# Aedelon/ProteinBERT-PyTorch-Replication

Hardware: AMD Instinct MI355X
Metric: sequences/sec (whole node) ProteinBERT pretrain L=512 at 1/2/4/8 MI355X (higher is better)
Workload: dtype bf16; 1 GPU; global_batch=2048, per_gpu_batch=2048, seq_len=512, parallelism=dp1, impl=hip, hip_graph=False

## Files before the change

proteinbert_pytorch_replication_amd/ops/csrc/lhead.hip:

```cpp
#include "mfma.h"

using namespace pbx;
typedef unsigned short bf16_t;

namespace {
constexpr int CH = 128;
constexpr int SB = 16;
constexpr int PT = 32;
constexpr int VP = 32;

__device__ __forceinline__ void stage_wo(unsigned char* wos, float* bo_s, const float* __restrict__ wo,
                                        const float* __restrict__ bo, int V) {
  for (int idx = threadIdx.x; idx < VP * 16; idx += blockDim.x) {
    const int v = idx >> 4, c8 = idx & 15;
    float e[8] = {0, 0, 0, 0, 0, 0, 0, 0};
    if (v < V) {
      const float4 a = *reinterpret_cast<const float4*>(wo + v * CH + c8 * 8);
      const float4 b = *reinterpret_cast<const float4*>(wo + v * CH + c8 * 8 + 4);
      e[0] = a.x; e[1] = a.y; e[2] = a.z; e[3] = a.w; e[4] = b.x; e[5] = b.y; e[6] = b.z; e[7] = b.w;
    }
    *reinterpret_cast<uint4*>(wos + swz256(v, c8)) = packq8(e);
  }
  if (threadIdx.x < VP) bo_s[threadIdx.x] = threadIdx.x < V ? bo[threadIdx.x] : 0.f;
}

__device__ __forceinline__ void tile_of(int L, int& b0, int& p0, int& chunk) {
  const int TP = (L + PT - 1) / PT;
  chunk = blockIdx.x / TP;
  b0 = chunk * SB;
  p0 = (blockIdx.x - chunk * TP) * PT;
}

__global__ void __launch_bounds__(512) lhead_logits_kernel(const bf16_t* __restrict__ h, const float* __restrict__ wo,
                                                           const float* __restrict__ bo, float* __restrict__ Z,
                                                           float2* __restrict__ part, int B, int L, int V) {
  extern __shared__ __attribute__((aligned(16))) unsigned char smem[];
  unsigned char* wos = smem;
  float* bo_s = reinterpret_cast<float*>(smem + VP * 256);
  float (*zt)[PT][VP + 1] = reinterpret_cast<float (*)[PT][VP + 1]>(bo_s + VP);
  const int tid = threadIdx.x, lane = tid & 63, w = tid >> 6;
  const int r = lane & 31, hh = lane >> 5;
  int b0, p0, chunk;
  tile_of(L, b0, p0, chunk);
  stage_wo(wos, bo_s, wo, bo, V);
  __syncthreads();
  bf16x8 wf[8];
#pragma unroll
  for (int kk = 0; kk < 8; ++kk) wf[kk] = lds_frag(wos, swz256(r, kk * 2 + hh));
  const float bv = bo_s[r];
#pragma unroll
  for (int si = 0; si < 2; ++si) {
    const int sl = 2 * w + si, b = b0 + sl;
    const int pos = p0 + r;
    const bool okrow = b < B && pos < L;
    const size_t row = (size_t)min(b, B - 1) * L + min(pos, L - 1);
    bf16x8 hf[8];
#pragma unroll
    for (int kk = 0; kk < 8; ++kk) hf[kk] = *reinterpret_cast<const bf16x8*>(h + row * CH + kk * 16 + 8 * hh);
    f32x16_t acc = zero16();
#pragma unroll
    for (int kk = 0; kk < 8; ++kk) acc = mfma32(hf[kk], wf[kk], acc);
#pragma unroll
    for (int e = 0; e < 16; ++e) {
      const int pl = (e & 3) + 8 * (e >> 2) + 4 * hh;
      const int pp = p0 + pl;
      const float z = acc[e] + bv;
      zt[sl][pl][r] = z;
      if (b < B && pp < L) Z[((size_t)b * L + pp) * VP + r] = r < V ? z : 0.f;
    }
    (void)okrow;
  }
  __syncthreads();
  {
    const int pl = tid >> 4, v0 = (tid & 15) * 2;
    const int pp = p0 + pl;
    const int nb = min(SB, B - b0);
    if (pp < L) {
#pragma unroll
      for (int j = 0; j < 2; ++j) {
        const int v = v0 + j;
        float m = -3.0e38f;
        for (int s = 0; s < nb; ++s) m = fmaxf(m, zt[s][pl][v]);
        float se = 0.f;
        for (int s = 0; s < nb; ++s) se += __expf(zt[s][pl][v] - m);
        part[((size_t)chunk * L + pp) * VP + v] = make_float2(m, se);
      }
    }
  }
}

__global__ void __launch_bounds__(256) lhead_fold_kernel(const float2* __restrict__ part, int nchunks, int L,
                                                         float2* __restrict__ out, int mode) {
  __shared__ float2 red[4][64];
  const int il = threadIdx.x & 63, cg = threadIdx.x >> 6;
  const int i = blockIdx.x * 64 + il;
  const bool ok = i < L * VP;
  float m = -3.0e38f, sum = 0.f;
  if (ok) {
    for (int c = cg; c < nchunks; c += 4) {
      const float2 p = part[(size_t)c * L * VP + i];
      if (mode != 1) {
        const float mn = fmaxf(m, p.x);
        sum = sum * __expf(m - mn) + p.y * __expf(p.x - mn);
        m = mn;
      } else {
        sum += p.x;
      }
    }
  }
  red[cg][il] = make_float2(m, sum);
  __syncthreads();
  if (cg != 0 || !ok) return;
  if (mode != 1) {
    float mm = red[0][il].x;
#pragma unroll
    for (int k = 1; k < 4; ++k) mm = fmaxf(mm, red[k][il].x);
    float ss = 0.f;
#pragma unroll
    for (int k = 0; k < 4; ++k) ss += red[k][il].y * __expf(red[k][il].x - mm);
    out[i] = make_float2(mm, mode == 2 ? ss : ss > 0.f ? 1.0f / ss : 0.f);
  } else {
    out[i] = make_float2(red[0][il].y + red[1][il].y + red[2][il].y + red[3][il].y, 0.f);
  }
}

struct RowTerms {
  float P[16], G[16];
  float loss;
};
__device__ __forceinline__ RowTerms row_terms(const float* __restrict__ Z, const float2* ms, size_t row, int pl,
                                              int hh, int V, bool ok, int yv, float coef) {
  RowTerms t;
  float zv[16];
  {
    const float4* zp0 = reinterpret_cast<const float4*>(Z + row * VP + 8 * hh);
    const float4* zp1 = reinterpret_cast<const float4*>(Z + row * VP + 16 + 8 * hh);
    const float4 a = zp0[0], b = zp0[1], c = zp1[0], d = zp1[1];
    const float tmp[16] = {a.x, a.y, a.z, a.w, b.x, b.y, b.z, b.w, c.x, c.y, c.z, c.w, d.x, d.y, d.z, d.w};
#pragma unroll
    for (int j = 0; j < 16; ++j) zv[j] = tmp[j];
  }
  float e[16], se = 0.f, py = 0.f;
#pragma unroll
  for (int j = 0; j < 16; ++j) {
    const int v = (j < 8 ? 0 : 16) + 8 * hh + (j & 7);
    const float2 s = ms[pl * VP + v];
    const bool inv = v < V;
    t.P[j] = inv ? __expf(zv[j] - s.x) * s.y : 0.f;
    e[j] = inv ? __expf(t.P[j]) : 0.f;
    se += e[j];
    py += v == yv ? t.P[j] : 0.f;
  }
  se += __shfl_xor(se, 32, 64);
  const float rse = 1.0f / se;
#pragma unroll
  for (int j = 0; j < 16; ++j) {
    const int v = (j < 8 ? 0 : 16) + 8 * hh + (j & 7);
    t.G[j] = ok ? coef * (e[j] * rse - (v == yv ? 1.f : 0.f)) : 0.f;
  }
  t.loss = ok ? ((hh == 0 ? __logf(se) : 0.f) - py) : 0.f;
  return t;
}

__global__ void __launch_bounds__(512) lhead_ce_kernel(const float* __restrict__ Z, const float2* __restrict__ MS,
                                                       const long long* __restrict__ y, const float* __restrict__ wl,
                                                       float2* __restrict__ tpart, float* __restrict__ loss_part,
                                                       int B, int L, int V, float inv_bl) {
  __shared__ float2 ms[PT * VP];
  __shared__ float gp[8][PT][VP + 1];
  __shared__ float red[8];
  const int tid = threadIdx.x, lane = tid & 63, w = tid >> 6;
  const int r = lane & 31, hh = lane >> 5;
  int b0, p0, chunk;
  tile_of(L, b0, p0, chunk);
  for (int i = tid; i < PT * VP; i += 512) {
    const int pp = min(p0 + i / VP, L - 1);
    ms[i] = MS[(size_t)pp * VP + (i % VP)];
  }
  __syncthreads();
  float acc[16];
#pragma unroll
  for (int j = 0; j < 16; ++j) acc[j] = 0.f;
  float lsum = 0.f;
#pragma unroll
  for (int si = 0; si < 2; ++si) {
    const int b = b0 + 2 * w + si, pos = p0 + r;
    const bool ok = b < B && pos < L;
    const size_t row = (size_t)min(b, B - 1) * L + min(pos, L - 1);
    const int yv = (int)y[row];
    const float wgt = ok ? wl[row] : 0.f;
    const RowTerms t = row_terms(Z, ms, row, r, hh, V, ok, yv, wgt * inv_bl);
    lsum += wgt * t.loss;
#pragma unroll
    for (int j = 0; j < 16; ++j) acc[j] += t.G[j] * t.P[j];
  }
#pragma unroll
  for (int j = 0; j < 16; ++j) gp[w][r][(j < 8 ? 0 : 16) + 8 * hh + (j & 7)] = acc[j];
  lsum = wave_reduce_sum(lsum);
  if (lane == 0) red[w] = lsum;
  __syncthreads();
  for (int i = tid; i < PT * VP; i += 512) {
    const int pl = i / VP, v = i % VP;
    if (p0 + pl < L) {
      float s = 0.f;
#pragma unroll
      for (int ww = 0; ww < 8; ++ww) s += gp[ww][pl][v];
      tpart[((size_t)chunk * L + p0 + pl) * VP + v] = make_float2(s, 0.f);
    }
  }
  if (tid == 0) {
    float s = 0.f;
#pragma unroll
    for (int ww = 0; ww < 8; ++ww) s += red[ww];
    loss_part[blockIdx.x] = s * inv_bl;
  }
}

__global__ void __launch_bounds__(512) lhead_grad_kernel(const float* __restrict__ Z, const float2* __restrict__ MS,
                                                         const float2* __restrict__ T, const long long* __restrict__ y,
                                                         const float* __restrict__ wl, const float* __restrict__ wo,
                                                         const float* __restrict__ bo, bf16_t* __restrict__ dh,
                                                         bf16_t* __restrict__ dz, float* __restrict__ dbo_part, int B,
                                                         int L, int V, float inv_bl) {
  extern __shared__ __attribute__((aligned(16))) unsigned char smem[];
  unsigned char* ot = smem;
  unsigned char* wos = smem + 8 * PT * 256;
  float2* ms = reinterpret_cast<float2*>(wos + VP * 256);
  float* ts = reinterpret_cast<float*>(ms + PT * VP);
  float* bo_s = ts + PT * VP;
  float (*dbr)[VP] = reinterpret_cast<float (*)[VP]>(bo_s + VP);
  const int tid = threadIdx.x, lane = tid & 63, w = tid >> 6;
  const int r = lane & 31, hh = lane >> 5;
  const int q = tr_q(lane), tc = tr_c(lane);
  int b0, p0, chunk;
  tile_of(L, b0, p0, chunk);
  stage_wo(wos, bo_s, wo, bo, V);
  for (int i = tid; i < PT * VP; i += 512) {
    const int pp = min(p0 + i / VP, L - 1);
    ms[i] = MS[(size_t)pp * VP + (i % VP)];
    ts[i] = T[(size_t)pp * VP + (i % VP)].x;
  }
  __syncthreads();
  float dba[16];
#pragma unroll
  for (int j = 0; j < 16; ++j) dba[j] = 0.f;
  unsigned char* myot = ot + w * PT * 256;
#pragma unroll 1
  for (int si = 0; si < 2; ++si) {
    const int b = b0 + 2 * w + si, pos = p0 + r;
    const bool ok = b < B && pos < L;
    const size_t row = (size_t)min(b, B - 1) * L + min(pos, L - 1);
    const int yv = (int)y[row];
    const float wgt = ok ? wl[row] : 0.f;
    const RowTerms t = row_terms(Z, ms, row, r, hh, V, ok, yv, wgt * inv_bl);
    float d[16];
#pragma unroll
    for (int j = 0; j < 16; ++j) {
      const int v = (j < 8 ? 0 : 16) + 8 * hh + (j & 7);
      d[j] = ok && v < V ? t.P[j] * (t.G[j] - ts[r * VP + v]) : 0.f;
      dba[j] += d[j];
    }
    const bf16x8 f0 = pack8(d), f1 = pack8(d + 8);
    if (ok) {
      *reinterpret_cast<bf16x8*>(dz + row * VP + 8 * hh) = f0;
      *reinterpret_cast<bf16x8*>(dz + row * VP + 16 + 8 * hh) = f1;
    }
    f32x16_t acc[4];
#pragma unroll
    for (int ct = 0; ct < 4; ++ct) acc[ct] = zero16();
#pragma unroll
    for (int kk = 0; kk < 2; ++kk) {
      const int rlo = kk * 16 + 8 * hh + q;
#pragma unroll
      for (int ct = 0; ct < 4; ++ct) {
        const int col = ct * 32 + tc;
        const bf16x8 fb = cat_tr(lds_tr(wos, swz256e(rlo, col)), lds_tr(wos, swz256e(rlo + 4, col)));
        acc[ct] = mfma32(kk == 0 ? f0 : f1, fb, acc[ct]);
      }
    }
#pragma unroll
    for (int ct = 0; ct < 4; ++ct)
#pragma unroll
      for (int e = 0; e < 16; ++e)
        *reinterpret_cast<bf16_t*>(myot + swz256e((e & 3) + 8 * (e >> 2) + 4 * hh, ct * 32 + r)) = f2bf(acc[ct][e]);
    __builtin_amdgcn_fence(__ATOMIC_RELEASE, "wavefront");
    __builtin_amdgcn_wave_barrier();
    __builtin_amdgcn_fence(__ATOMIC_ACQUIRE, "wavefront");
    if (b < B) {
#pragma unroll
      for (int i = 0; i < 8; ++i) {
        const int idx = lane + 64 * i;
        const int rr = idx >> 4, c8 = idx & 15;
        if (p0 + rr < L)
          *reinterpret_cast<uint4*>(dh + ((size_t)b * L + p0 + rr) * CH + c8 * 8) =
              *reinterpret_cast<const uint4*>(myot + swz256(rr, c8));
      }
    }
    __builtin_amdgcn_fence(__ATOMIC_RELEASE, "wavefront");
    __builtin_amdgcn_wave_barrier();
    __builtin_amdgcn_fence(__ATOMIC_ACQUIRE, "wavefront");
  }
#pragma unroll
  for (int j = 0; j < 16; ++j) {
#pragma unroll
    for (int o = 1; o < 32; o <<= 1) dba[j] += __shfl_xor(dba[j], o, 64);
  }
  if (r == 0) {
#pragma unroll
    for (int j = 0; j < 16; ++j) dbr[w][(j < 8 ? 0 : 16) + 8 * hh + (j & 7)] = dba[j];
  }
  __syncthreads();
  if (tid < V) {
    float s = 0.f;
#pragma unroll
    for (int ww = 0; ww < 8; ++ww) s += dbr[ww][tid];
    dbo_part[(size_t)blockIdx.x * V + tid] = s;
  }
}

constexpr int ROWSF = 1024;
constexpr int ZS = VP + 1;
constexpr int FUSED_LDS = ROWSF * ZS * 4 + VP * 256 + VP * 4 + 8 * 64 * 8 + 64 * 8 + 64 * 4 + 8 * 4;

template <int PP>
__global__ void __launch_bounds__(512) lhead_fused_kernel(const bf16_t* __restrict__ h, const float* __restrict__ wo,
                                                          const float* __restrict__ bo,
                                                          const long long* __restrict__ y,
                                                          const float* __restrict__ wl, bf16_t* __restrict__ dh,
                                                          bf16_t* __restrict__ dz, float* __restrict__ dbo_part,
                                                          float* __restrict__ loss_part, int B, int L, int V,
                                                          float inv_bl) {
  extern __shared__ __attribute__((aligned(16))) unsigned char smem[];
  constexpr int NPAIR = PP * 32, PARTS = 512 / NPAIR;
  float* zt = reinterpret_cast<float*>(smem);
  unsigned char* wos = smem + ROWSF * ZS * 4;
  float* bo_s = reinterpret_cast<float*>(wos + VP * 256);
  float2* red = reinterpret_cast<float2*>(bo_s + VP);
  float2* ms = red + 8 * 64;
  float* tt = reinterpret_cast<float*>(ms + 64);
  float* lred = tt + 64;
  const int tid = threadIdx.x, lane = tid & 63, w = tid >> 6;
  const int r = lane & 31, hh = lane >> 5;
  const int q = tr_q(lane), tc = tr_c(lane);
  const int l0 = blockIdx.x * PP;
  const int NR = PP * B, NT = (NR + 31) / 32;
  stage_wo(wos, bo_s, wo, bo, V);
  __syncthreads();
  {
    bf16x8 wf[8];
#pragma unroll
    for (int kk = 0; kk < 8; ++kk) wf[kk] = lds_frag(wos, swz256(r, kk * 2 + hh));
    const float bv = bo_s[r];
#pragma unroll 2
    for (int t = w; t < NT; t += 8) {
      const int row = min(t * 32 + r, NR - 1);
      const int p = row / B, s = row - (row / B) * B;
      const bf16_t* src = h + ((size_t)s * L + min(l0 + p, L - 1)) * CH + 8 * hh;
      bf16x8 hf[8];
#pragma unroll
      for (int kk = 0; kk < 8; ++kk) hf[kk] = *reinterpret_cast<const bf16x8*>(src + kk * 16);
      f32x16_t acc = zero16();
#pragma unroll
      for (int kk = 0; kk < 8; ++kk) acc = mfma32(hf[kk], wf[kk], acc);
#pragma unroll
      for (int e = 0; e < 16; ++e) {
        const int rr = t * 32 + (e & 3) + 8 * (e >> 2) + 4 * hh;
        if (rr < NR) zt[rr * ZS + r] = acc[e] + bv;
      }
    }
  }
  __syncthreads();
  const int pair = tid % NPAIR, part = tid / NPAIR;
  const int pp = pair >> 5, pv = pair & 31;
  {
    float m = -3.0e38f, se = 0.f;
    for (int s = part; s < B; s += PARTS) {
      const float z = zt[(pp * B + s) * ZS + pv];
      const float mn = fmaxf(m, z);
      se = se * __expf(m - mn) + __expf(z - mn);
      m = mn;
    }
    red[part * NPAIR + pair] = make_float2(m, se);
  }
  __syncthreads();
  if (tid < NPAIR) {
    float mm = red[tid].x;
#pragma unroll
    for (int k = 1; k < PARTS; ++k) mm = fmaxf(mm, red[k * NPAIR + tid].x);
    float ss = 0.f;
#pragma unroll
    for (int k = 0; k < PARTS; ++k) ss += red[k * NPAIR + tid].y * __expf(red[k * NPAIR + tid].x - mm);
    ms[tid] = make_float2(mm, ss > 0.f ? 1.0f / ss : 0.f);
  }
  __syncthreads();
  constexpr int RPT = ROWSF / 512;
  float P[RPT][VP], rse[RPT], coef[RPT];
  int yv[RPT];
  float lsum = 0.f;
#pragma unroll
  for (int k = 0; k < RPT; ++k) {
    const int row = tid + 512 * k;
    const int p = min(row / B, PP - 1), s = row - (row / B) * B;
    const bool ok = row < NR && l0 + p < L;
    const size_t gi = (size_t)s * L + min(l0 + p, L - 1);
    yv[k] = ok ? (int)y[gi] : -1;
    const float wgt = ok ? wl[gi] : 0.f;
    coef[k] = wgt * inv_bl;
    float e[VP], se = 0.f, py = 0.f;
#pragma unroll
    for (int v = 0; v < VP; ++v) {
      const float2 mv = ms[p * 32 + v];
      const float z = row < NR ? zt[row * ZS + v] : 0.f;
      P[k][v] = ok && v < V ? __expf(z - mv.x) * mv.y : 0.f;
      e[v] = ok && v < V ? __expf(P[k][v]) : 0.f;
      se += e[v];
      py += v == yv[k] ? P[k][v] : 0.f;
    }
    rse[k] = se > 0.f ? 1.0f / se : 0.f;
    lsum += ok ? wgt * (__logf(se) - py) : 0.f;
    if (row < NR) {
#pragma unroll
      for (int v = 0; v < VP; ++v) zt[row * ZS + v] = coef[k] * (e[v] * rse[k] - (v == yv[k] ? 1.f : 0.f)) * P[k][v];
    }
  }
  __syncthreads();
  {
    float a = 0.f;
    for (int s = part; s < B; s += PARTS) a += zt[(pp * B + s) * ZS + pv];
    red[part * NPAIR + pair] = make_float2(a, 0.f);
  }
  __syncthreads();
  if (tid < NPAIR) {
    float a = 0.f;
#pragma unroll
    for (int k = 0; k < PARTS; ++k) a += red[k * NPAIR + tid].x;
    tt[tid] = a;
  }
  __syncthreads();
#pragma unroll
  for (int k = 0; k < RPT; ++k) {
    const int row = tid + 512 * k;
    if (row >= NR) continue;
    const int p = row / B, s = row - (row / B) * B;
    const bool ok = l0 + p < L;
    float d[VP];
#pragma unroll
    for (int v = 0; v < VP; ++v) {
      const float G = coef[k] * (__expf(P[k][v]) * rse[k] - (v == yv[k] ? 1.f : 0.f));
      d[v] = ok && v < V ? P[k][v] * (G - tt[p * 32 + v]) : 0.f;
      zt[row * ZS + v] = d[v];
    }
    if (ok) {
      uint4* dst = reinterpret_cast<uint4*>(dz + ((size_t)s * L + l0 + p) * VP);
#pragma unroll
      for (int c = 0; c < 4; ++c) dst[c] = packq8(d + 8 * c);
    }
  }
  lsum = wave_reduce_sum(lsum);
  if (lane == 0) lred[w] = lsum;
  __syncthreads();
  if (tid == 0) {
    float a = 0.f;
#pragma unroll
    for (int k = 0; k < 8; ++k) a += lred[k];
    loss_part[blockIdx.x] = a * inv_bl;
  }
  {
    const int v = tid & 31, sl = tid >> 5;
    float a = 0.f;
    for (int row = sl; row < NR; row += 16) a += zt[row * ZS + v];
    reinterpret_cast<float*>(red)[sl * 32 + v] = a;
  }
  constexpr int TPW = ROWSF / 32 / 8;
  bf16x8 fa[TPW][2];
#pragma unroll
  for (int i = 0; i < TPW; ++i) {
    const int row = (w + 8 * i) * 32 + r;
#pragma unroll
    for (int kk = 0; kk < 2; ++kk) {
      float a8[8];
#pragma unroll
      for (int j = 0; j < 8; ++j) a8[j] = row < NR ? zt[row * ZS + kk * 16 + 8 * hh + j] : 0.f;
      fa[i][kk] = pack8(a8);
    }
  }
  __syncthreads();
  if (tid < V) {
    float a = 0.f;
#pragma unroll
    for (int sl = 0; sl < 16; ++sl) a += reinterpret_cast<float*>(red)[sl * 32 + tid];
    dbo_part[(size_t)blockIdx.x * V + tid] = a;
  }
  unsigned char* myot = smem + w * PT * 256;
#pragma unroll
  for (int i = 0; i < TPW; ++i) {
    const int t = w + 8 * i;
    if (t >= NT) break;
    f32x16_t acc[4];
#pragma unroll
    for (int ct = 0; ct < 4; ++ct) acc[ct] = zero16();
#pragma unroll
    for (int kk = 0; kk < 2; ++kk) {
      const int rlo = kk * 16 + 8 * hh + q;
#pragma unroll
      for (int ct = 0; ct < 4; ++ct) {
        const int col = ct * 32 + tc;
        const bf16x8 fb = cat_tr(lds_tr(wos, swz256e(rlo, col)), lds_tr(wos, swz256e(rlo + 4, col)));
        acc[ct] = mfma32(fa[i][kk], fb, acc[ct]);
      }
    }
#pragma unroll
    for (int ct = 0; ct < 4; ++ct)
#pragma unroll
      for (int e = 0; e < 16; ++e)
        *reinterpret_cast<bf16_t*>(myot + swz256e((e & 3) + 8 * (e >> 2) + 4 * hh, ct * 32 + r)) = f2bf(acc[ct][e]);
    __builtin_amdgcn_fence(__ATOMIC_RELEASE, "wavefront");
    __builtin_amdgcn_wave_barrier();
    __builtin_amdgcn_fence(__ATOMIC_ACQUIRE, "wavefront");
#pragma unroll
    for (int k = 0; k < 8; ++k) {
      const int idx = lane + 64 * k;
      const int rr = idx >> 4, c8 = idx & 15;
      const int row = t * 32 + rr;
      const int p = row / B, s = row - (row / B) * B;
      if (row < NR && l0 + p < L)
        *reinterpret_cast<uint4*>(dh + ((size_t)s * L + l0 + p) * CH + c8 * 8) =
            *reinterpret_cast<const uint4*>(myot + swz256(rr, c8));
    }
    __builtin_amdgcn_fence(__ATOMIC_RELEASE, "wavefront");
    __builtin_amdgcn_wave_barrier();
    __builtin_amdgcn_fence(__ATOMIC_ACQUIRE, "wavefront");
  }
}
}

PBX_EXPORT int pbx_local_head3_tiles(int B, int L) { return ((B + SB - 1) / SB) * ((L + PT - 1) / PT); }

namespace {
constexpr int LDS1 = VP * 256 + VP * 4 + SB * PT * (VP + 1) * 4;
constexpr int LDS5 = 8 * PT * 256 + VP * 256 + PT * VP * 8 + PT * VP * 4 + VP * 4 + 8 * VP * 4;
void lhead3_attrs() {
  static bool attr = false;
  if (!attr) {
    (void)hipFuncSetAttribute((const void*)lhead_logits_kernel, hipFuncAttributeMaxDynamicSharedMemorySize, LDS1);
    (void)hipFuncSetAttribute((const void*)lhead_grad_kernel, hipFuncAttributeMaxDynamicSharedMemorySize, LDS5);
    attr = true;
  }
}
}

PBX_EXPORT int pbx_local_head3_a(const void* h, const float* wo, const float* bo, float* Z, float* part, float* MS,
                                 int raw, int B, int L, int V, hipStream_t st) {
  if (V > VP || V < 1 || B < 1 || L < 1) return (int)hipErrorInvalidValue;
  lhead3_attrs();
  const int nt = pbx_local_head3_tiles(B, L);
  const int nch = (B + SB - 1) / SB;
  hipLaunchKernelGGL(lhead_logits_kernel, dim3(nt), dim3(512), LDS1, st, (const bf16_t*)h, wo, bo, Z, (float2*)part,
                     B, L, V);
  hipLaunchKernelGGL(lhead_fold_kernel, dim3((L * VP + 63) / 64), dim3(256), 0, st, (const float2*)part, nch, L,
                     (float2*)MS, raw ? 2 : 0);
  return pbx_launch_status();
}

PBX_EXPORT int pbx_local_head3_b(const float* Z, const float* MS, const void* y, const float* wl, float* tpart,
                                 float* loss_part, float* T, int B, int L, int V, hipStream_t st) {
  if (V > VP || V < 1 || B < 1 || L < 1) return (int)hipErrorInvalidValue;
  const int nt = pbx_local_head3_tiles(B, L);
  const int nch = (B + SB - 1) / SB;
  const float inv_bl = 1.0f / ((float)B * (float)L);
  hipLaunchKernelGGL(lhead_ce_kernel, dim3(nt), dim3(512), 0, st, Z, (const float2*)MS, (const long long*)y, wl,
                     (float2*)tpart, loss_part, B, L, V, inv_bl);
  hipLaunchKernelGGL(lhead_fold_kernel, dim3((L * VP + 63) / 64), dim3(256), 0, st, (const float2*)tpart, nch, L,
                     (float2*)T, 1);
  return pbx_launch_status();
}

PBX_EXPORT int pbx_local_head3_c(const float* Z, const float* MS, const float* T, const void* y, const float* wl,
                                 const float* wo, const float* bo, void* dh, void* dz, float* dbo_part, int B, int L,
                                 int V, hipStream_t st) {
  if (V > VP || V < 1 || B < 1 || L < 1) return (int)hipErrorInvalidValue;
  lhead3_attrs();
  const int nt = pbx_local_head3_tiles(B, L);
  const float inv_bl = 1.0f / ((float)B * (float)L);
  hipLaunchKernelGGL(lhead_grad_kernel, dim3(nt), dim3(512), LDS5, st, Z, (const float2*)MS, (const float2*)T,
                     (const long long*)y, wl, wo, bo, (bf16_t*)dh, (bf16_t*)dz, dbo_part, B, L, V, inv_bl);
  return pbx_launch_status();
}

PBX_EXPORT int pbx_local_head3(const void* h, const float* wo, const float* bo, const void* y, const float* wl,
                               void* dh, void* dz, float* dbo_part, float* loss_part, float* Z, float* part,
                               float* tpart, float* MS, float* T, int B, int L, int V, hipStream_t st) {
  int rc = pbx_local_head3_a(h, wo, bo, Z, part, MS, 0, B, L, V, st);
  if (rc == 0) rc = pbx_local_head3_b(Z, MS, y, wl, tpart, loss_part, T, B, L, V, st);
  if (rc == 0) rc = pbx_local_head3_c(Z, MS, T, y, wl, wo, bo, dh, dz, dbo_part, B, L, V, st);
  return rc;
}

PBX_EXPORT int pbx_local_head_fused_pp(int B) { return B <= 512 ? 2 : B <= 1024 ? 1 : 0; }

PBX_EXPORT int pbx_local_head_fused(const void* h, const float* wo, const float* bo, const void* y, const float* wl,
                                    void* dh, void* dz, float* dbo_part, float* loss_part, int B, int L, int V,
                                    hipStream_t st) {
  const int pp = pbx_local_head_fused_pp(B);
  if (V > VP || V < 1 || B < 1 || pp == 0 || L < 1) return (int)hipErrorInvalidValue;
  static bool attr = false;
  if (!attr) {
    (void)hipFuncSetAttribute((const void*)lhead_fused_kernel<2>, hipFuncAttributeMaxDynamicSharedMemorySize, FUSED_LDS);
    (void)hipFuncSetAttribute((const void*)lhead_fused_kernel<1>, hipFuncAttributeMaxDynamicSharedMemorySize, FUSED_LDS);
    attr = true;
  }
  const float inv_bl = 1.0f / ((float)B * (float)L);
  hipLaunchKernelGGL(pp == 2 ? lhead_fused_kernel<2> : lhead_fused_kernel<1>, dim3((L + pp - 1) / pp), dim3(512),
                     FUSED_LDS, st, (const bf16_t*)h, wo, bo, (const long long*)y, wl, (bf16_t*)dh, (bf16_t*)dz,
                     dbo_part, loss_part, B, L, V, inv_bl);
  return pbx_launch_status();
}
```

proteinbert_pytorch_replication_amd/ops/global_track.py:

```python
from __future__ import annotations

import ctypes
from typing import Dict, List, Optional, Tuple

import torch

from . import _lib, streams
from .gemm import gemm as _gemm, gemm_batch
from .gemm import go_head_parts
from ..parallel import batch_softmax
from ..train.arena import notify_grads_ready
from ..utils.determinism import fused_deterministic

_P, _I, _F = ctypes.c_void_p, ctypes.c_int, ctypes.c_float
_lib.register("pbx_row_ln_fwd", [_P, _P, _P, _P, _I, _P, _I, _P, _P, _P, _P, _P, _P, _P, _I, _I, _F, _P])
_lib.register("pbx_row_ln_bwd", [_P, _P, _P, _P, _P, _P, _P, _P, _P, _P, _P, _P, _P, _I, _P, _P, _I, _I, _P])
_lib.register("pbx_bias_gelu", [_P, _P, _P, _P, _I, _I, _P])
_lib.register("pbx_bias_gelu_bwd", [_P, _P, _P, _P, _P, _I, _I, _P, _P])
_lib.register("pbx_colsum_add", [_P, _I, _I, _P, _P, _P])
_lib.register("pbx_colsum_set", [_P, _I, _I, _P, _P, _P])
_lib.register("pbx_local_head3", [_P, _P, _P, _P, _P, _P, _P, _P, _P, _P, _P, _P, _P, _P, _I, _I, _I, _P])
_lib.register("pbx_local_head3_tiles", [_I, _I])
_lib.register("pbx_local_head_fused", [_P, _P, _P, _P, _P, _P, _P, _P, _P, _I, _I, _I, _P])
_lib.register("pbx_local_head3_a", [_P, _P, _P, _P, _P, _P, _I, _I, _I, _I, _P])
_lib.register("pbx_local_head3_b", [_P, _P, _P, _P, _P, _P, _P, _I, _I, _I, _P])
_lib.register("pbx_local_head3_c", [_P, _P, _P, _P, _P, _P, _P, _P, _P, _P, _I, _I, _I, _P])
LHEAD_FUSED = True


def local_head_forward(h: torch.Tensor, wo: torch.Tensor, bo: torch.Tensor, y_l: torch.Tensor, w_l: torch.Tensor,
                       loss_slot: torch.Tensor):
    dev = h.device
    st = _s(dev)
    B, L, C = h.shape
    V = wo.shape[0]
    if batch_softmax.active():
        return _local_head_dp(h, wo, bo, y_l, w_l, loss_slot)
    if LHEAD_FUSED and B <= 1024:
        pp = _lib.lib().pbx_local_head_fused_pp(B)
        nt = (L + pp - 1) // pp
        dh = torch.empty_like(h)
        dz = torch.empty((B * L, 32), dtype=BF16, device=dev)
        dbo_part = torch.empty((nt, V), dtype=F32, device=dev)
        lparts = torch.empty(nt, dtype=F32, device=dev)
        _lib.call("pbx_local_head_fused", h.data_ptr(), wo.detach().contiguous().data_ptr(), bo.data_ptr(),
                  y_l.contiguous().data_ptr(), w_l.float().contiguous().data_ptr(), dh.data_ptr(), dz.data_ptr(),
                  dbo_part.data_ptr(), lparts.data_ptr(), B, L, V, st)
        _lib.call("pbx_colsum_set", lparts.data_ptr(), nt, 1, loss_slot.data_ptr(), None, st)
        return dh, dz, dbo_part
    nt = _lib.lib().pbx_local_head3_tiles(B, L)
    nch = (B + 15) // 16
    dh = torch.empty_like(h)
    dz = torch.empty((B * L, 32), dtype=BF16, device=dev)
    dbo_part = torch.empty((nt, V), dtype=F32, device=dev)
    lparts = torch.empty(nt, dtype=F32, device=dev)
    Z = torch.empty((B * L, 32), dtype=F32, device=dev)
    part = torch.empty((2, nch, L, 32, 2), dtype=F32, device=dev)
    ms_t = torch.empty((2, L, 32, 2), dtype=F32, device=dev)
    _lib.call("pbx_local_head3", h.data_ptr(), wo.detach().contiguous().data_ptr(), bo.data_ptr(),
              y_l.contiguous().data_ptr(), w_l.float().contiguous().data_ptr(), dh.data_ptr(), dz.data_ptr(),
              dbo_part.data_ptr(), lparts.data_ptr(), Z.data_ptr(), part[0].data_ptr(), part[1].data_ptr(),
              ms_t[0].data_ptr(), ms_t[1].data_ptr(), B, L, V, st)
    _lib.call("pbx_colsum_set", lparts.data_ptr(), nt, 1, loss_slot.data_ptr(), None, st)
    return dh, dz, dbo_part


def _local_head_dp(h, wo, bo, y_l, w_l, loss_slot):
    dev = h.device
    st = _s(dev)
    B, L, C = h.shape
    V = wo.shape[0]
    nt = _lib.lib().pbx_local_head3_tiles(B, L)
    nch = (B + 15) // 16
    dh = torch.empty_like(h)
    dz = torch.empty((B * L, 32), dtype=BF16, device=dev)
    dbo_part = torch.empty((nt, V), dtype=F32, device=dev)
    lparts = torch.empty(nt, dtype=F32, device=dev)
    Z = torch.empty((B * L, 32), dtype=F32, device=dev)
    part = torch.empty((2, nch, L, 32, 2), dtype=F32, device=dev)
    ms_t = torch.empty((2, L, 32, 2), dtype=F32, device=dev)
    wo_c = wo.detach().contiguous()
    y_c = y_l.contiguous()
    w_c = w_l.float().contiguous()
    _lib.call("pbx_local_head3_a", h.data_ptr(), wo_c.data_ptr(), bo.data_ptr(), Z.data_ptr(), part[0].data_ptr(),
              ms_t[0].data_ptr(), 1, B, L, V, st)
    batch_softmax.merge_head_stats(ms_t[0])
    _lib.call("pbx_local_head3_b", Z.data_ptr(), ms_t[0].data_ptr(), y_c.data_ptr(), w_c.data_ptr(),
              part[1].data_ptr(), lparts.data_ptr(), ms_t[1].data_ptr(), B, L, V, st)
    batch_softmax.all_reduce_(ms_t[1], "sum")
    _lib.call("pbx_local_head3_c", Z.data_ptr(), ms_t[0].data_ptr(), ms_t[1].data_ptr(), y_c.data_ptr(),
              w_c.data_ptr(), wo_c.data_ptr(), bo.data_ptr(), dh.data_ptr(), dz.data_ptr(), dbo_part.data_ptr(),
              B, L, V, st)
    _lib.call("pbx_colsum_set", lparts.data_ptr(), nt, 1, loss_slot.data_ptr(), None, st)
    return dh, dz, dbo_part


_lib.register("pbx_glob_bwd", [_P, _I, _I, _I, _I, _P, _P])
_lib.register("pbx_glob3_fwd", [_P, _I, _I, _I, _I, _I, _F, _P])
_lib.register("pbx_pack_glob_frags", [_P, _P, _P, _I, _I, _P])

LN_EPS = 1e-5
BF16 = torch.bfloat16
F32 = torch.float32


def _p(t: Optional[torch.Tensor]):
    return None if t is None else t.data_ptr()


def _s(dev) -> int:
    return _lib.stream_ptr(dev)


def bf16_of(p: torch.Tensor) -> torch.Tensor:
    v = getattr(p, "_pbx_bf16", None)
    if v is not None:
        if p._version != p._pbx_bf16_ver:
            with torch.no_grad():
                v.data.copy_(p.detach())
            p._pbx_bf16_ver = p._version
        return v
    return p.detach().to(BF16)


def _operand(t: torch.Tensor, inner_axis: int):
    if t.stride(1) == 1:
        return t, False
    if t.stride(0) == 1:
        return t.t(), True
    return t.contiguous(), False


def mm32(a: torch.Tensor, b: torch.Tensor) -> torch.Tensor:
    out = torch.empty((a.shape[0], b.shape[1]), dtype=F32, device=a.device)
    (a0, ta), (b0, tb) = _operand(a, 1), _operand(b, 1)
    return _gemm(a0, b0, out, ta, tb)


def addmm_into(dst: torch.Tensor, a: torch.Tensor, b: torch.Tensor) -> None:
    (a0, ta), (b0, tb) = _operand(a, 1), _operand(b, 1)
    _gemm(a0, b0, dst, ta, tb, accumulate=True)


def addmm_new(c: torch.Tensor, a: torch.Tensor, b: torch.Tensor) -> torch.Tensor:
    out = c.float().clone()
    addmm_into(out, a, b)
    return out


A_ALIGN = 8


def padded_cols(n: int) -> int:
    return (n + A_ALIGN - 1) // A_ALIGN * A_ALIGN


_PAD_CACHE = {}


def bf16_padded(p: torch.Tensor) -> torch.Tensor:
    R, Cc = p.shape
    key = (id(p), p.device)
    buf = _PAD_CACHE.get(key)
    if buf is None or buf.shape != (R, padded_cols(Cc)):
        buf = torch.zeros((R, padded_cols(Cc)), dtype=BF16, device=p.device)
        _PAD_CACHE[key] = buf
    view = buf[:, :Cc]
    view.copy_(bf16_of(p))
    return view


class _Grads:

    def __init__(self, params):
        self.params = params
        self.dst: List[torch.Tensor] = []
        self.direct: List[bool] = []
        for p in params:
            g = getattr(p, "grad", None) if getattr(p, "_pbx_arena", False) else None
            if g is not None and g.is_contiguous() and g.dtype == F32:
                self.dst.append(g)
                self.direct.append(True)
            elif p is not None and not p.requires_grad:
                self.dst.append(_scratch_like(p))
                self.direct.append(False)
            else:
                self.dst.append(None if p is None else torch.zeros(p.shape, dtype=F32, device=p.device))
                self.direct.append(False)

    def finish(self):
        direct = [p for p, d in zip(self.params, self.direct) if d and p is not None]
        if direct:
            notify_grads_ready(direct)
        return [None if (d or p is None or not p.requires_grad) else g
                for p, g, d in zip(self.params, self.dst, self.direct)]


_SCRATCH: Dict[Tuple, torch.Tensor] = {}


def _scratch_like(p: torch.Tensor) -> torch.Tensor:
    key = (tuple(p.shape), str(p.device))
    t = _SCRATCH.get(key)
    if t is None:
        t = torch.empty(p.shape, dtype=F32, device=p.device)
        _SCRATCH[key] = t
    return t


_lib.register("pbx_ann_supported", [_I, _I, _I])
_lib.register("pbx_ann_csr", [_P, _I, _I, _P, _P, _P])
_lib.register("pbx_ann_wt", [_P, _P, _I, _I, _P])
_lib.register("pbx_ann_fwd", [_P, _P, _P, _P, _P, _P, _P, _I, _I, _I, _P])
_lib.register("pbx_ann_csc", [_P, _I, _I, _P, _P, _P, _P])
_lib.register("pbx_ann_wgrad", [_P, _P, _P, _P, _P, _P, _P, _P, _I, _I, _I, _P])
ANN_SPARSE = True


def ann_sparse_ok(B: int, A: int, G: int) -> bool:
    return ANN_SPARSE and bool(_lib.lib().pbx_ann_supported(B, A, G))


class InputLayerFn(torch.autograd.Function):

    @staticmethod
    def forward(ctx, ann, w, b, wgl, bgl):
        dev = ann.device
        st = _s(dev)
        B, A = ann.shape
        G = w.shape[0]
        sparse = ann_sparse_ok(B, A, G)
        if sparse:
            annc = ann.float().contiguous()
            train = any(ctx.needs_input_grad)
            aux = train and streams.ENABLED and dev.type == "cuda"
            wt = torch.empty((A, G), dtype=BF16, device=dev)
            wd = w.detach().contiguous()
            if aux:
                with streams.on_aux(dev, "ann", keep=[annc, wd, wt]):
                    _lib.call("pbx_ann_wt", wd.data_ptr(), wt.data_ptr(), G, A, _s(dev))
            else:
                _lib.call("pbx_ann_wt", wd.data_ptr(), wt.data_ptr(), G, A, st)
            cnt = torch.empty(B, dtype=torch.int32, device=dev)
            ent = torch.empty((B * A, 2), dtype=torch.int32, device=dev)
            _lib.call("pbx_ann_csr", annc.data_ptr(), B, A, cnt.data_ptr(), ent.data_ptr(), st)
            if aux:
                streams.wait_for(dev, "ann")
            u = torch.empty((B, G), dtype=F32, device=dev)
            g = torch.empty_like(u)
            g_bf = torch.empty((B, G), dtype=BF16, device=dev)
            _lib.call("pbx_ann_fwd", cnt.data_ptr(), ent.data_ptr(), wt.data_ptr(), b.detach().contiguous().data_ptr(),
                      u.data_ptr(), g.data_ptr(), g_bf.data_ptr(), B, A, G, st)
            saved_x = None
            if train:
                ccnt = torch.empty(A, dtype=torch.int32, device=dev)
                cptr = torch.empty(A, dtype=torch.int32, device=dev)
                cent = torch.empty(((A + 63) // 64 * 64 * B, 2), dtype=torch.int32, device=dev)
                if aux:
                    with streams.on_aux(dev, "ann", keep=[annc, ccnt, cptr, cent]):
                        _lib.call("pbx_ann_csc", annc.data_ptr(), B, A, ccnt.data_ptr(), cptr.data_ptr(),
                                  cent.data_ptr(), _s(dev))
                    streams.mark_ready(dev, "ann", [ccnt])
                else:
                    _lib.call("pbx_ann_csc", annc.data_ptr(), B, A, ccnt.data_ptr(), cptr.data_ptr(), cent.data_ptr(),
                              st)
                ctx.csc = (ccnt, cptr, cent, A)
        else:
            ann_pad = torch.empty((B, padded_cols(A)), dtype=BF16, device=dev)
            ann_pad[:, A:].zero_()
            ann_bf = ann_pad[:, :A]
            ann_bf.copy_(ann)
            wp = bf16_padded(w)
            u = torch.empty((B, G), dtype=F32, device=dev)
            _gemm(ann_bf, wp, u, ta=False, tb=True, pad_a=True, pad_b=True)
            g = torch.empty_like(u)
            g_bf = torch.empty((B, G), dtype=BF16, device=dev)
            _lib.call("pbx_bias_gelu", u.data_ptr(), b.data_ptr(), g.data_ptr(), g_bf.data_ptr(), B, G, st)
            saved_x = ann_bf
        ugl = mm32(g_bf, bf16_of(wgl).t())
        gb = torch.empty_like(ugl)
        _lib.call("pbx_bias_gelu", ugl.data_ptr(), bgl.data_ptr(), gb.data_ptr(), None, B, ugl.shape[1], st)
        ctx.save_for_backward(saved_x, u, g_bf, ugl)
        ctx.params = (w, b, wgl, bgl)
        ctx.sparse = sparse
        ctx.mark_non_differentiable(g_bf)
        ctx.set_materialize_grads(False)
        return g, g_bf, gb

    @staticmethod
    def backward(ctx, dg, _dgbf, dgb):
        saved = ctx.saved_tensors
        dev = saved[1].device
        early = dev.type == "cuda" and streams.forked(dev, "ann")
        if early and not all(_Grads(list(ctx.params)).direct):
            streams.cancel_fork(dev, "ann")
            early = False
        if early:
            extra = list(ctx.csc[:3]) if getattr(ctx, "csc", None) is not None else []
            with streams.on_aux(dev, "ann", keep=[*saved, dg, dgb, *extra]) as scope:
                out = InputLayerFn._backward(ctx, saved, dg, dgb)
                scope.keep(*[t for t in out if isinstance(t, torch.Tensor)])
            return out
        return InputLayerFn._backward(ctx, saved, dg, dgb)

    @staticmethod
    def _backward(ctx, saved, dg, dgb):
        x, u, g_bf, ugl = saved
        w, b, wgl, bgl = ctx.params
        dev = u.device
        st = _s(dev)
        B, G = u.shape
        gr = _Grads([w, b, wgl, bgl])
        dw, db, dwgl, dbgl = gr.dst
        dg = torch.zeros((B, G), dtype=F32, device=dev) if dg is None else dg.float().contiguous()
        if dgb is not None:
            N = ugl.shape[1]
            dugl = torch.empty((B, N), dtype=BF16, device=dev)
            _lib.call("pbx_bias_gelu_bwd", dgb.float().contiguous().data_ptr(), ugl.data_ptr(), bgl.data_ptr(),
                      dugl.data_ptr(), dbgl.data_ptr(), B, N, _lib.ptr(_det_slab(min(B, BGB_ROWS), N, dev)), st)
            addmm_into(dwgl, dugl.t(), g_bf)
            dg = addmm_new(dg, dugl, bf16_of(wgl))
        if ctx.sparse:
            ccnt, cptr, cent, A = ctx.csc
            streams.wait_ready(ccnt)
            streams.queue_join()
            dut = torch.empty((G, B), dtype=F32, device=dev)
            _lib.call("pbx_ann_wgrad", dg.data_ptr(), u.data_ptr(), ccnt.data_ptr(), cptr.data_ptr(), cent.data_ptr(),
                      dut.data_ptr(), dw.data_ptr(), db.data_ptr(), B, A, G, st)
            del ctx.csc
            return (None, *gr.finish())
        du = torch.empty((B, G), dtype=BF16, device=dev)
        _lib.call("pbx_bias_gelu_bwd", dg.data_ptr(), u.data_ptr(), b.data_ptr(), du.data_ptr(), db.data_ptr(), B, G,
                  _lib.ptr(_det_slab(min(B, BGB_ROWS), G, dev)), st)
        _gemm(du, x, dw, ta=True, tb=False, accumulate=True, pad_b=True)
        return (None, *gr.finish())


BGB_ROWS = 256


def _det_slab(rows: int, cols: int, dev) -> Optional[torch.Tensor]:
    return torch.empty((rows, cols), dtype=F32, device=dev) if fused_deterministic() else None
# ... 360 lines not shown
```

Measured before the change: 107,500 sequences/s.

## Replace LDS-staged fused local head with register-resident one-pass kernel up to B=2048

```diff
diff --git a/proteinbert_pytorch_replication_amd/ops/csrc/lhead.hip b/proteinbert_pytorch_replication_amd/ops/csrc/lhead.hip
--- a/proteinbert_pytorch_replication_amd/ops/csrc/lhead.hip
+++ b/proteinbert_pytorch_replication_amd/ops/csrc/lhead.hip
@@ -318,202 +318,232 @@
   }
 }
 
-constexpr int ROWSF = 1024;
-constexpr int ZS = VP + 1;
-constexpr int FUSED_LDS = ROWSF * ZS * 4 + VP * 256 + VP * 4 + 8 * 64 * 8 + 64 * 8 + 64 * 4 + 8 * 4;
-
-template <int PP>
-__global__ void __launch_bounds__(512) lhead_fused_kernel(const bf16_t* __restrict__ h, const float* __restrict__ wo,
-                                                          const float* __restrict__ bo,
-                                                          const long long* __restrict__ y,
-                                                          const float* __restrict__ wl, bf16_t* __restrict__ dh,
-                                                          bf16_t* __restrict__ dz, float* __restrict__ dbo_part,
-                                                          float* __restrict__ loss_part, int B, int L, int V,
-                                                          float inv_bl) {
+constexpr int OP_RING = 2;
+constexpr int OP_OTS = 272;
+constexpr int OP_LDS = 8 * PT * OP_OTS + VP * 256 + VP * 4 + 8 * VP * 8 + VP * 8 + VP * 4 + 8 * 4;
+static_assert(2 * OP_LDS <= 160 * 1024, "two workgroups per CU");
+
+template <int TPW>
+__global__ void __launch_bounds__(512) lhead_onepass_kernel(const bf16_t* __restrict__ h, const float* __restrict__ wo,
+                                                            const float* __restrict__ bo,
+                                                            const long long* __restrict__ y,
+                                                            const float* __restrict__ wl, bf16_t* __restrict__ dh,
+                                                            bf16_t* __restrict__ dz, float* __restrict__ dbo_part,
+                                                            float* __restrict__ loss_part, int B, int L, int V,
+                                                            float inv_bl) {
   extern __shared__ __attribute__((aligned(16))) unsigned char smem[];
-  constexpr int NPAIR = PP * 32, PARTS = 512 / NPAIR;
-  float* zt = reinterpret_cast<float*>(smem);
-  unsigned char* wos = smem + ROWSF * ZS * 4;
+  unsigned char* ot = smem;
+  unsigned char* wos = smem + 8 * PT * OP_OTS;
   float* bo_s = reinterpret_cast<float*>(wos + VP * 256);
   float2* red = reinterpret_cast<float2*>(bo_s + VP);
-  float2* ms = red + 8 * 64;
-  float* tt = reinterpret_cast<float*>(ms + 64);
-  float* lred = tt + 64;
-  const int tid = threadIdx.x, lane = tid & 63, w = tid >> 6;
+  float2* ms = red + 8 * VP;
+  float* tred = reinterpret_cast<float*>(red);
+  float* dbr = tred + 8 * VP;
+  float* tt = reinterpret_cast<float*>(ms + VP);
+  float* lred = tt + VP;
+  const int tid = threadIdx.x, lane = tid & 63;
+  const int w = __builtin_amdgcn_readfirstlane(tid >> 6);
   const int r = lane & 31, hh = lane >> 5;
   const int q = tr_q(lane), tc = tr_c(lane);
-  const int l0 = blockIdx.x * PP;
-  const int NR = PP * B, NT = (NR + 31) / 32;
+  const int l = blockIdx.x;
+  const int NT = (B + 31) >> 5;
+  bf16x8 ring[OP_RING][8];
+  auto load_tile = [&](bf16x8 (&dst)[8], int t) {
+    const int s = min(t * 32 + r, B - 1);
+    const bf16_t* src = h + ((size_t)s * L + l) * CH + 8 * hh;
+#pragma unroll
+    for (int kk = 0; kk < 8; ++kk) dst[kk] = *reinterpret_cast<const bf16x8*>(src + kk * 16);
+  };
+#pragma unroll
+  for (int i = 0; i < OP_RING && i < TPW; ++i)
+    if (w + 8 * i < NT) load_tile(ring[i], w + 8 * i);
   stage_wo(wos, bo_s, wo, bo, V);
   __syncthreads();
+  float Z[TPW][16];
   {
     bf16x8 wf[8];
 #pragma unroll
     for (int kk = 0; kk < 8; ++kk) wf[kk] = lds_frag(wos, swz256(r, kk * 2 + hh));
-    const float bv = bo_s[r];
-#pragma unroll 2
-    for (int t = w; t < NT; t += 8) {
-      const int row = min(t * 32 + r, NR - 1);
-      const int p = row / B, s = row - (row / B) * B;
-      const bf16_t* src = h + ((size_t)s * L + min(l0 + p, L - 1)) * CH + 8 * hh;
-      bf16x8 hf[8];
-#pragma unroll
-      for (int kk = 0; kk < 8; ++kk) hf[kk] = *reinterpret_cast<const bf16x8*>(src + kk * 16);
+#pragma unroll
+    for (int i = 0; i < TPW; ++i) {
+      const int t = w + 8 * i;
       f32x16_t acc = zero16();
-#pragma unroll
-      for (int kk = 0; kk < 8; ++kk) acc = mfma32(hf[kk], wf[kk], acc);
-#pragma unroll
-      for (int e = 0; e < 16; ++e) {
-        const int rr = t * 32 + (e & 3) + 8 * (e >> 2) + 4 * hh;
-        if (rr < NR) zt[rr * ZS + r] = acc[e] + bv;
+      if (t < NT) {
+#pragma unroll
+        for (int kk = 0; kk < 8; ++kk) acc = mfma32(wf[kk], ring[i % OP_RING][kk], acc);
+        if (i + OP_RING < TPW && t + 8 * OP_RING < NT) load_tile(ring[i % OP_RING], t + 8 * OP_RING);
       }
-    }
-  }
-  __syncthreads();
-  const int pair = tid % NPAIR, part = tid / NPAIR;
-  const int pp = pair >> 5, pv = pair & 31;
+#pragma unroll
+      for (int e = 0; e < 16; ++e) Z[i][e] = acc[e];
+    }
+  }
+  float m[16], f[16];
   {
-    float m = -3.0e38f, se = 0.f;
-    for (int s = part; s < B; s += PARTS) {
-      const float z = zt[(pp * B + s) * ZS + pv];
-      const float mn = fmaxf(m, z);
-      se = se * __expf(m - mn) + __expf(z - mn);
-      m = mn;
-    }
-    red[part * NPAIR + pair] = make_float2(m, se);
-  }
-  __syncthreads();
-  if (tid < NPAIR) {
+    const float4* bp = reinterpret_cast<const float4*>(bo_s + 4 * hh);
+#pragma unroll
+    for (int g = 0; g < 4; ++g) {
+      const float4 b4 = bp[2 * g];
+      f[4 * g] = b4.x; f[4 * g + 1] = b4.y; f[4 * g + 2] = b4.z; f[4 * g + 3] = b4.w;
+    }
+  }
+#pragma unroll
+  for (int e = 0; e < 16; ++e) m[e] = -3.0e38f;
+#pragma unroll
+  for (int i = 0; i < TPW; ++i) {
+    const bool ok = (w + 8 * i) * 32 + r < B;
+#pragma unroll
+    for (int e = 0; e < 16; ++e) {
+      Z[i][e] = ok ? Z[i][e] + f[e] : -3.0e38f;
+      m[e] = fmaxf(m[e], Z[i][e]);
+    }
+  }
+#pragma unroll
+  for (int e = 0; e < 16; ++e) {
+#pragma unroll
+    for (int o = 1; o < 32; o <<= 1) m[e] = fmaxf(m[e], __shfl_xor(m[e], o, 64));
+  }
+#pragma unroll
+  for (int e = 0; e < 16; ++e) f[e] = 0.f;
+#pragma unroll
+  for (int i = 0; i < TPW; ++i) {
+    const bool ok = (w + 8 * i) * 32 + r < B;
+#pragma unroll
+    for (int e = 0; e < 16; ++e) {
+      Z[i][e] = ok ? __expf(Z[i][e] - m[e]) : 0.f;
+      f[e] += Z[i][e];
+    }
+  }
+#pragma unroll
+  for (int e = 0; e < 16; ++e) {
+#pragma unroll
+    for (int o = 1; o < 32; o <<= 1) f[e] += __shfl_xor(f[e], o, 64);
+  }
+  if (r == 0) {
+#pragma unroll
+    for (int e = 0; e < 16; ++e) red[w * VP + (e & 3) + 8 * (e >> 2) + 4 * hh] = make_float2(m[e], f[e]);
+  }
+  int yv[TPW];
+  float wg[TPW];
+#pragma unroll
+  for (int i = 0; i < TPW; ++i) {
+    const int s = (w + 8 * i) * 32 + r;
+    const size_t gi = (size_t)min(s, B - 1) * L + l;
+    const long long yr = y[gi];
+    const float wr = wl[gi];
+    yv[i] = s < B ? (int)yr : -1;
+    wg[i] = s < B ? wr : 0.f;
+  }
+  __syncthreads();
+  if (tid < VP) {
     float mm = red[tid].x;
 #pragma unroll
-    for (int k = 1; k < PARTS; ++k) mm = fmaxf(mm, red[k * NPAIR + tid].x);
+    for (int k = 1; k < 8; ++k) mm = fmaxf(mm, red[k * VP + tid].x);
     float ss = 0.f;
 #pragma unroll
-    for (int k = 0; k < PARTS; ++k) ss += red[k * NPAIR + tid].y * __expf(red[k * NPAIR + tid].x - mm);
-    ms[tid] = make_float2(mm, ss > 0.f ? 1.0f / ss : 0.f);
-  }
-  __syncthreads();
-  constexpr int RPT = ROWSF / 512;
-  float P[RPT][VP], rse[RPT], coef[RPT];
-  int yv[RPT];
-  float lsum = 0.f;
-#pragma unroll
-  for (int k = 0; k < RPT; ++k) {
-    const int row = tid + 512 * k;
-    const int p = min(row / B, PP - 1), s = row - (row / B) * B;
-    const bool ok = row < NR && l0 + p < L;
-    const size_t gi = (size_t)s * L + min(l0 + p, L - 1);
-    yv[k] = ok ? (int)y[gi] : -1;
-    const float wgt = ok ? wl[gi] : 0.f;
-    coef[k] = wgt * inv_bl;
-    float e[VP], se = 0.f, py = 0.f;
-#pragma unroll
-    for (int v = 0; v < VP; ++v) {
-      const float2 mv = ms[p * 32 + v];
-      const float z = row < NR ? zt[row * ZS + v] : 0.f;
-      P[k][v] = ok && v < V ? __expf(z - mv.x) * mv.y : 0.f;
-      e[v] = ok && v < V ? __expf(P[k][v]) : 0.f;
-      se += e[v];
-      py += v == yv[k] ? P[k][v] : 0.f;
-    }
-    rse[k] = se > 0.f ? 1.0f / se : 0.f;
-    lsum += ok ? wgt * (__logf(se) - py) : 0.f;
-    if (row < NR) {
-#pragma unroll
-      for (int v = 0; v < VP; ++v) zt[row * ZS + v] = coef[k] * (e[v] * rse[k] - (v == yv[k] ? 1.f : 0.f)) * P[k][v];
-    }
-  }
-  __syncthreads();
-  {
+    for (int k = 0; k < 8; ++k) ss += red[k * VP + tid].y * __expf(red[k * VP + tid].x - mm);
+    ms[tid] = make_float2(mm, tid < V && ss > 0.f ? 1.0f / ss : 0.f);
+  }
+  __syncthreads();
+#pragma unroll
+  for (int e = 0; e < 16; ++e) {
+    const float2 mv = ms[(e & 3) + 8 * (e >> 2) + 4 * hh];
+    f[e] = __expf(m[e] - mv.x) * mv.y;
+  }
+#pragma unroll
+  for (int i = 0; i < TPW; ++i)
+#pragma unroll
+    for (int e = 0; e < 16; ++e) Z[i][e] *= f[e];
+  float lse[TPW], lsum = 0.f;
+#pragma unroll
+  for (int e = 0; e < 16; ++e) f[e] = 0.f;
+#pragma unroll
+  for (int i = 0; i < TPW; ++i) {
+    float ex[16], se = 0.f, py = 0.f;
+#pragma unroll
+    for (int e = 0; e < 16; ++e) {
+      const int v = (e & 3) + 8 * (e >> 2) + 4 * hh;
+      ex[e] = v < V ? __expf(Z[i][e]) : 0.f;
+      se += ex[e];
+      py += v == yv[i] ? Z[i][e] : 0.f;
+    }
+    se += __shfl_xor(se, 32, 64);
+    const float rse = 1.0f / se;
+    lse[i] = __logf(se);
+    const float coef = wg[i] * inv_bl;
+    lsum += wg[i] * ((hh == 0 ? lse[i] : 0.f) - py);
+#pragma unroll
+    for (int e = 0; e < 16; ++e) {
+      const int v = (e & 3) + 8 * (e >> 2) + 4 * hh;
+      f[e] += coef * (ex[e] * rse - (v == yv[i] ? 1.f : 0.f)) * Z[i][e];
+    }
+  }
+#pragma unroll
+  for (int e = 0; e < 16; ++e) {
+#pragma unroll
+    for (int o = 1; o < 32; o <<= 1) f[e] += __shfl_xor(f[e], o, 64);
+  }
+  lsum = wave_reduce_sum(lsum);
+  if (r == 0) {
+#pragma unroll
+    for (int e = 0; e < 16; ++e) tred[w * VP + (e & 3) + 8 * (e >> 2) + 4 * hh] = f[e];
+  }
+  if (lane == 0) lred[w] = lsum;
+  __syncthreads();
+  if (tid < VP) {
     float a = 0.f;
-    for (int s = part; s < B; s += PARTS) a += zt[(pp * B + s) * ZS + pv];
-    red[part * NPAIR + pair] = make_float2(a, 0.f);
-  }
-  __syncthreads();
-  if (tid < NPAIR) {
-    float a = 0.f;
-#pragma unroll
-    for (int k = 0; k < PARTS; ++k) a += red[k * NPAIR + tid].x;
+#pragma unroll
+    for (int k = 0; k < 8; ++k) a += tred[k * VP + tid];
     tt[tid] = a;
   }
-  __syncthreads();
-#pragma unroll
-  for (int k = 0; k < RPT; ++k) {
-    const int row = tid + 512 * k;
-    if (row >= NR) continue;
-    const int p = row / B, s = row - (row / B) * B;
-    const bool ok = l0 + p < L;
-    float d[VP];
-#pragma unroll
-    for (int v = 0; v < VP; ++v) {
-      const float G = coef[k] * (__expf(P[k][v]) * rse[k] - (v == yv[k] ? 1.f : 0.f));
-      d[v] = ok && v < V ? P[k][v] * (G - tt[p * 32 + v]) : 0.f;
-      zt[row * ZS + v] = d[v];
-    }
-    if (ok) {
-      uint4* dst = reinterpret_cast<uint4*>(dz + ((size_t)s * L + l0 + p) * VP);
-#pragma unroll
-      for (int c = 0; c < 4; ++c) dst[c] = packq8(d + 8 * c);
-    }
-  }
-  lsum = wave_reduce_sum(lsum);
-  if (lane == 0) lred[w] = lsum;
-  __syncthreads();
   if (tid == 0) {
     float a = 0.f;
 #pragma unroll
     for (int k = 0; k < 8; ++k) a += lred[k];
-    loss_part[blockIdx.x] = a * inv_bl;
-  }
-  {
-    const int v = tid & 31, sl = tid >> 5;
-    float a = 0.f;
-    for (int row = sl; row < NR; row += 16) a += zt[row * ZS + v];
-    reinterpret_cast<float*>(red)[sl * 32 + v] = a;
-  }
-  constexpr int TPW = ROWSF / 32 / 8;
-  bf16x8 fa[TPW][2];
-#pragma unroll
-  for (int i = 0; i < TPW; ++i) {
-    const int row = (w + 8 * i) * 32 + r;
-#pragma unroll
-    for (int kk = 0; kk < 2; ++kk) {
-      float a8[8];
-#pragma unroll
-      for (int j = 0; j < 8; ++j) a8[j] = row < NR ? zt[row * ZS + kk * 16 + 8 * hh + j] : 0.f;
-      fa[i][kk] = pack8(a8);
-    }
-  }
-  __syncthreads();
-  if (tid < V) {
-    float a = 0.f;
-#pragma unroll
-    for (int sl = 0; sl < 16; ++sl) a += reinterpret_cast<float*>(red)[sl * 32 + tid];
-    dbo_part[(size_t)blockIdx.x * V + tid] = a;
-  }
-  unsigned char* myot = smem + w * PT * 256;
+    loss_part[l] = a * inv_bl;
+  }
+  __syncthreads();
+#pragma unroll
+  for (int e = 0; e < 16; ++e) {
+    m[e] = tt[(e & 3) + 8 * (e >> 2) + 4 * hh];
+    f[e] = 0.f;
+  }
+  unsigned char* myot = ot + w * PT * OP_OTS;
 #pragma unroll
   for (int i = 0; i < TPW; ++i) {
     const int t = w + 8 * i;
     if (t >= NT) break;
-    f32x16_t acc[4];
-#pragma unroll
-    for (int ct = 0; ct < 4; ++ct) acc[ct] = zero16();
-#pragma unroll
-    for (int kk = 0; kk < 2; ++kk) {
-      const int rlo = kk * 16 + 8 * hh + q;
-#pragma unroll
-      for (int ct = 0; ct < 4; ++ct) {
-        const int col = ct * 32 + tc;
-        const bf16x8 fb = cat_tr(lds_tr(wos, swz256e(rlo, col)), lds_tr(wos, swz256e(rlo + 4, col)));
-        acc[ct] = mfma32(fa[i][kk], fb, acc[ct]);
+    const int s = t * 32 + r;
+    const float coef = wg[i] * inv_bl;
+    const int yl = yv[i] - 4 * hh;
+    float d[16];
+#pragma unroll
+    for (int e = 0; e < 16; ++e) {
+      const float ge = coef * __expf(Z[i][e] - lse[i]);
+      const float G = (e & 3) + 8 * (e >> 2) == yl ? ge - coef : ge;
+      d[e] = Z[i][e] * (G - m[e]);
+      f[e] += d[e];
+    }
+    if (s < B) {
+      bf16_t* dst = dz + ((size_t)s * L + l) * VP + 4 * hh;
+#pragma unroll
+      for (int g = 0; g < 4; ++g) *reinterpret_cast<uint2*>(dst + 8 * g) = packq4(d + 4 * g);
+    }
+    const bf16x8 fa[2] = {pack8(d), pack8(d + 8)};
+#pragma unroll
+    for (int ct = 0; ct < 4; ++ct) {
+      f32x16_t acc = zero16();
+#pragma unroll
+      for (int kk = 0; kk < 2; ++kk) {
+        const int rlo = kk * 16 + 4 * hh + q, col = ct * 32 + tc;
+        const bf16x8 fb = cat_tr(lds_tr(wos, swz256e(rlo, col)), lds_tr(wos, swz256e(rlo + 8, col)));
+        acc = mfma32(fb, fa[kk], acc);
       }
-    }
-#pragma unroll
-    for (int ct = 0; ct < 4; ++ct)
-#pragma unroll
-      for (int e = 0; e < 16; ++e)
-        *reinterpret_cast<bf16_t*>(myot + swz256e((e & 3) + 8 * (e >> 2) + 4 * hh, ct * 32 + r)) = f2bf(acc[ct][e]);
+#pragma unroll
+      for (int g = 0; g < 4; ++g) {
+        const float o4[4] = {acc[4 * g], acc[4 * g + 1], acc[4 * g + 2], acc[4 * g + 3]};
+        *reinterpret_cast<uint2*>(myot + r * OP_OTS + 8 * hh + (ct * 4 + g) * 16) = packq4(o4);
+      }
+    }
     __builtin_amdgcn_fence(__ATOMIC_RELEASE, "wavefront");
     __builtin_amdgcn_wave_barrier();
     __builtin_amdgcn_fence(__ATOMIC_ACQUIRE, "wavefront");
@@ -521,15 +551,30 @@
     for (int k = 0; k < 8; ++k) {
       const int idx = lane + 64 * k;
       const int rr = idx >> 4, c8 = idx & 15;
-      const int row = t * 32 + rr;
-      const int p = row / B, s = row - (row / B) * B;
-      if (row < NR && l0 + p < L)
-        *reinterpret_cast<uint4*>(dh + ((size_t)s * L + l0 + p) * CH + c8 * 8) =
-            *reinterpret_cast<const uint4*>(myot + swz256(rr, c8));
+      const int sr = t * 32 + rr;
+      if (sr < B)
+        *reinterpret_cast<uint4*>(dh + ((size_t)sr * L + l) * CH + c8 * 8) =
+            *reinterpret_cast<const uint4*>(myot + rr * OP_OTS + c8 * 16);
     }
     __builtin_amdgcn_fence(__ATOMIC_RELEASE, "wavefront");
     __builtin_amdgcn_wave_barrier();
     __builtin_amdgcn_fence(__ATOMIC_ACQUIRE, "wavefront");
+  }
+#pragma unroll
+  for (int e = 0; e < 16; ++e) {
+#pragma unroll
+    for (int o = 1; o < 32; o <<= 1) f[e] += __shfl_xor(f[e], o, 64);
+  }
+  if (r == 0) {
+#pragma unroll
+    for (int e = 0; e < 16; ++e) dbr[w * VP + (e & 3) + 8 * (e >> 2) + 4 * hh] = f[e];
+  }
+  __syncthreads();
+  if (tid < V) {
+    float a = 0.f;
+#pragma unroll
+    for (int k = 0; k < 8; ++k) a += dbr[k * VP + tid];
+    dbo_part[(size_t)l * V + tid] = a;
   }
 }
 }
@@ -596,22 +641,22 @@
   return rc;
 }
 
-PBX_EXPORT int pbx_local_head_fused_pp(int B) { return B <= 512 ? 2 : B <= 1024 ? 1 : 0; }
+PBX_EXPORT int pbx_local_head_fused_pp(int B) { return B >= 1 && B <= 2048 ? 1 : 0; }
 
 PBX_EXPORT int pbx_local_head_fused(const void* h, const float* wo, const float* bo, const void* y, const float* wl,
                                     void* dh, void* dz, float* dbo_part, float* loss_part, int B, int L, int V,
                                     hipStream_t st) {
-  const int pp = pbx_local_head_fused_pp(B);
-  if (V > VP || V < 1 || B < 1 || pp == 0 || L < 1) return (int)hipErrorInvalidValue;
+  if (V > VP || V < 1 || pbx_local_head_fused_pp(B) == 0 || L < 1) return (int)hipErrorInvalidValue;
   static bool attr = false;
   if (!attr) {
-    (void)hipFuncSetAttribute((const void*)lhead_fused_kernel<2>, hipFuncAttributeMaxDynamicSharedMemorySize, FUSED_LDS);
-    (void)hipFuncSetAttribute((const void*)lhead_fused_kernel<1>, hipFuncAttributeMaxDynamicSharedMemorySize, FUSED_LDS);
+    (void)hipFuncSetAttribute((const void*)lhead_onepass_kernel<8>, hipFuncAttributeMaxDynamicSharedMemorySize, OP_LDS);
+    (void)hipFuncSetAttribute((const void*)lhead_onepass_kernel<4>, hipFuncAttributeMaxDynamicSharedMemorySize, OP_LDS);
+    (void)hipFuncSetAttribute((const void*)lhead_onepass_kernel<2>, hipFuncAttributeMaxDynamicSharedMemorySize, OP_LDS);
     attr = true;
   }
   const float inv_bl = 1.0f / ((float)B * (float)L);
-  hipLaunchKernelGGL(pp == 2 ? lhead_fused_kernel<2> : lhead_fused_kernel<1>, dim3((L + pp - 1) / pp), dim3(512),
-                     FUSED_LDS, st, (const bf16_t*)h, wo, bo, (const long long*)y, wl, (bf16_t*)dh, (bf16_t*)dz,
-                     dbo_part, loss_part, B, L, V, inv_bl);
+  auto k = B <= 512 ? lhead_onepass_kernel<2> : B <= 1024 ? lhead_onepass_kernel<4> : lhead_onepass_kernel<8>;
+  hipLaunchKernelGGL(k, dim3(L), dim3(512), OP_LDS, st, (const bf16_t*)h, wo, bo, (const long long*)y, wl,
+                     (bf16_t*)dh, (bf16_t*)dz, dbo_part, loss_part, B, L, V, inv_bl);
   return pbx_launch_status();
 }
diff --git a/proteinbert_pytorch_replication_amd/ops/global_track.py b/proteinbert_pytorch_replication_amd/ops/global_track.py
--- a/proteinbert_pytorch_replication_amd/ops/global_track.py
+++ b/proteinbert_pytorch_replication_amd/ops/global_track.py
@@ -26,6 +26,7 @@
 _lib.register("pbx_local_head3_b", [_P, _P, _P, _P, _P, _P, _P, _I, _I, _I, _P])
 _lib.register("pbx_local_head3_c", [_P, _P, _P, _P, _P, _P, _P, _P, _P, _P, _I, _I, _I, _P])
 LHEAD_FUSED = True
+LHEAD_FUSED_MAX_B = 2048
 
 
 def local_head_forward(h: torch.Tensor, wo: torch.Tensor, bo: torch.Tensor, y_l: torch.Tensor, w_l: torch.Tensor,
@@ -36,8 +37,8 @@
     V = wo.shape[0]
     if batch_softmax.active():
         return _local_head_dp(h, wo, bo, y_l, w_l, loss_slot)
-    if LHEAD_FUSED and B <= 1024:
-        pp = _lib.lib().pbx_local_head_fused_pp(B)
+    pp = _lib.lib().pbx_local_head_fused_pp(B) if LHEAD_FUSED and B <= LHEAD_FUSED_MAX_B else 0
+    if pp:
         nt = (L + pp - 1) // pp
         dh = torch.empty_like(h)
         dz = torch.empty((B * L, 32), dtype=BF16, device=dev)
```

After: 109,000 sequences/s, median of 6. 1.01x the previous value.
